# kkrt-labs/stwo-brainfuck

Hardware: AMD Instinct MI355X
Metric: trace cells committed+proved/sec (higher is better)
Workload: dtype u32 (M31 / QM31 modular arithmetic)

## Files before the change

stwo-brainfuck_amd/csrc/api.hip:

```cpp
#include "../../include/bfhip.h"
#include "ctx.h"
#include <cstdlib>
#include "host/circle.h"
#include "host/quotients.h"
#include "host/hash.h"
#include <cstdio>
#include <vector>
#include <algorithm>
#include <chrono>

using namespace bf;

static thread_local std::string g_err;
void bfhip_set_error(const std::string& s) { g_err = s; }

#define API_TRY try {
#define API_CTX(ctx) try { if (!(ctx)) throw HipError("null context"); (ctx)->c.bind();
#define API_CATCH } catch (const std::exception& e) { g_err = e.what(); return -1; } catch (...) { g_err = "unknown error"; return -1; }

namespace bf {

void Ctx::ensure_aux() { for (auto& a : aux) if (!a) BF_HIP(hipStreamCreateWithFlags(&a, hipStreamNonBlocking)); }
void Ctx::ensure_side() { if (!stream2) BF_HIP(hipStreamCreateWithFlags(&stream2, hipStreamNonBlocking)); }

// ... 817 lines not shown
        total = q_add(total, claimed[k]);
        reports[k] = check_report_init();
    }
    CheckLaunch launches[N_COMPONENTS];
    const CheckLaunch* d_launches = nullptr;
    CheckReportDev* d_reports = nullptr;
    {
        StageBatch sb(c);
        d_reports = c.stage(reports, N_COMPONENTS);
        for (int k = 0; k < N_COMPONENTS; k++) launches[k] = check_launch_of(k, log_sizes[k], rows[k], inter[k], el, claimed[k], d_reports + k);
        d_launches = c.stage(launches, N_COMPONENTS);
        sb.end();
    }
    {
        ProfScope ps(c.stream, "k_check_cells", 0);
        for (int k = 0; k < N_COMPONENTS; k++) check_constraints_launch(c.stream, k, d_launches + k, log_sizes[k]);
    }
    BF_HIP(hipGetLastError());
    c.read_back(reports, d_reports, sizeof reports);
    int32_t n_bad = 0;
    for (int k = 0; k < N_COMPONENTS; k++) { check_report_fill(out[k], reports[k], k, log_sizes[k], claimed[k]); n_bad += reports[k].n_bad_cells != 0; }
    logup_total_h[0] = total.a.a; logup_total_h[1] = total.a.b; logup_total_h[2] = total.b.a; logup_total_h[3] = total.b.b;
    if (n_bad_components) *n_bad_components = n_bad;
    return 0;
    API_CATCH
}
int32_t bfhip_accumulate_quotients(bfhip_ctx* ctx, uint32_t log_size, const uint32_t* const* cols_h, const uint32_t* col_shifts_h, uint32_t n_cols,
                                   const uint32_t* n_samples_h, const uint32_t* sample_points_h, const uint32_t* sample_values_h,
                                   const uint32_t random_coeff_h[4], uint32_t* const out_d[4]) {
    API_CTX(ctx)
    Ctx& c = ctx->c;
    if (log_size < 3 || log_size > c.tw_root_log + 1) throw HipError("accumulate_quotients: log_size outside the twiddle tree");
    std::vector<ColDesc> descs(n_cols);
    std::vector<std::vector<ColumnSample>> samples(n_cols);
    size_t si = 0;
    for (u32 k = 0; k < n_cols; k++) {
        descs[k] = ColDesc{cols_h[k], col_shifts_h ? col_shifts_h[k] : 0u, 0};
        if (descs[k].shift == 1) throw HipError("accumulate_quotients: column shift must be 0 or >= 2");
        for (u32 s = 0; s < n_samples_h[k]; s++, si++) {
            const uint32_t* p = sample_points_h + 8 * si;
            samples[k].push_back({PtQ{q_from_h(p), q_from_h(p + 4)}, q_from_h(sample_values_h + 4 * si)});
        }
    }
    std::vector<QuotientBatch> batches; std::vector<QuotientEntry> entries;
    build_quotient_batches(samples, q_from_h(random_coeff_h), batches, entries);
    quotient_entries_finish(batches.data(), batches.size(), entries.data(), descs.data());
    c.stage_checkpoint();
    QuotientArgs a{};
    a.batches = batches.empty() ? nullptr : c.stage(batches.data(), batches.size());
    a.entries = entries.empty() ? nullptr : c.stage(entries.data(), entries.size());
    a.n_batches = (u32)batches.size(); a.log = log_size; a.tw = c.d_tw; a.tw_total = 1u << c.tw_root_log;
    for (int w = 0; w < 4; w++) a.out[w] = out_d[w];
    const u32 blocks = quotient_groups_layout(&a, 1);
    accumulate_quotients(c.stream, c.stage(&a, 1), 1, blocks);
    BF_HIP(hipGetLastError());
    return 0;
    API_CATCH
}

}

#ifdef BFHIP_TEST_HOOKS
__global__ void __launch_bounds__(256) k_test_field_op(u32 op, const u32* __restrict__ a, const u32* __restrict__ b, u32* __restrict__ out, u32 n) {
    const u32 i = blockIdx.x * blockDim.x + threadIdx.x;
    if (i >= n) return;
    const u32 a0 = a[4 * i], a1 = a[4 * i + 1], a2 = a[4 * i + 2], a3 = a[4 * i + 3];
    const u32 b0 = b[4 * i], b1 = b[4 * i + 1], b2 = b[4 * i + 2], b3 = b[4 * i + 3];
    const u64 a64 = ((u64)a1 << 32) | a0;
    const Q31 x = q_make(a0, a1, a2, a3), y = q_make(b0, b1, b2, b3);
    Q31 r = q_zero();
    switch (op) {
        case 0: r.a.a = m_add(a0, b0); break;
        case 1: r.a.a = m_sub(a0, b0); break;
        case 2: r.a.a = m_mul(a0, b0); break;
        case 3: r.a.a = m_mul_pre2(a0, 2u * b0); break;
        case 4: r.a.a = m_mul_pow2(a0, b0 % 31u); break;
        case 5: r.a.a = m_inv(a0); break;
        case 6: r.a.a = m_red4(a64); break;
        case 7: r.a.a = m_canon(a64); break;
        case 8: r = q_mul(x, y); break;
        case 9: r = q_mul_const(x, q_const(y)); break;
        default: r = q_inv(x); break;
    }
    out[4 * i] = r.a.a; out[4 * i + 1] = r.a.b; out[4 * i + 2] = r.b.a; out[4 * i + 3] = r.b.b;
}
extern "C" int32_t bfhip_test_field_op(bfhip_ctx* ctx, uint32_t op, const uint32_t* a_d, const uint32_t* b_d, uint32_t* out_d, size_t n) {
    API_CTX(ctx)
    if (op > 10) throw HipError("bfhip_test_field_op: unknown op");
    if (!a_d || !b_d || !out_d) throw HipError("null argument");
    if (n == 0 || n > (size_t(1) << 28)) throw HipError("bfhip_test_field_op: n out of range");
    hipLaunchKernelGGL(k_test_field_op, dim3((u32)((n + 255) / 256)), dim3(256), 0, ctx->c.stream, op, a_d, b_d, out_d, (u32)n);
    BF_HIP(hipGetLastError());
    return 0;
    API_CATCH
}
extern "C" int32_t bfhip_test_constraint_group_rows(int32_t component, uint32_t log_size, uint32_t main_shift) {
    if (component < 0 || component >= N_COMPONENTS) { g_err = "unknown component"; return -1; }
    ConstraintLaunch L{};
    for (u32 j = 0; j < n_main_cols(component); j++) L.trace[j].shift = main_shift;
    for (u32 j = 0; j + 4 < 4 * n_logup_cols(component); j++) L.inter[j].shift = main_shift;
    L.log_size = log_size;
    return (int32_t)constraint_group_rows(L, component);
}
#endif
```

stwo-brainfuck_amd/csrc/kernels.h:

```cpp
#pragma once
#include <hip/hip_runtime.h>
#include "m31.h"
#include "air.h"
#include <string>
#include <vector>

struct bfhip_trace;

namespace bf {

struct ColDesc { const u32* ptr; u32 shift; u32 pad_; };

int prof_mode(hipStream_t s);
void prof_enable(hipStream_t s, int mode);
void prof_run_begin(hipStream_t s, const char* name);
void prof_run_end(hipStream_t s);
void prof_begin(hipStream_t s, const char* name, double bytes, double units, double aux = 0.0);
void prof_end(hipStream_t s);
void prof_reset(hipStream_t s);
std::string prof_report_json(const hipStream_t* streams, int n);
void prof_forget(hipStream_t s);
struct ProfScope {
    hipStream_t s; bool on;
    ProfScope(hipStream_t s_, const char* name, double bytes, double units = 0.0, bool dominant = false, double aux = 0.0) : s(s_) {
// ... 80 lines not shown
    const u32* src[4]; const u32* quot[4]; u32* dst[4]; uint4* tree[18];
    const u32* alpha8; const u32* itw; u32 tw_total, log, rfc, pad_;
    u32* counter; u32* chan; u32* alpha_out; u32* root_out;
};
void fri_layer(hipStream_t stream, const FriLayerArgs& a);
void grind_span(hipStream_t stream, const u32* d_digest, u64 base, u32 span, u32 pow_bits, unsigned long long* d_best, u32 mix_u64_conv);
void clock_probe_launch(hipStream_t stream, uint4* d_stamps, u32* d_sink, u32 blocks, u32 iters);
void clock_sampler_launch(hipStream_t stream, uint4* d_out, const u32* d_stop_alias, unsigned long long max_ticks);
void fill_mix(hipStream_t stream, u32* p, size_t n);
void channel_mix_root_draw(hipStream_t stream, u32* d_chan, const u32* d_root, u32* d_alpha8, u32* d_root_copy);

void merkle_layer_poseidon(hipStream_t stream, void* out, const void* prev, const ColDesc* d_cols, u32 ncols, u32 log, u32 out_shift = 0, u32 prev_shift = 0,
                           u32 first = 0, u32 count = 0);
void hades_once(hipStream_t stream, const u32* d_in24, u32* d_out24);

struct ConstraintLaunch {
    const u32* is_first; ColDesc trace[13]; ColDesc inter[12]; u32* acc[4]; Q31 coeff[12]; Lookups el; Q31 total_sum; u32 denom_inv[2]; u32 log_size;
    u32 overwrite;
    u32 row0, n_rows;
    const u32* inter_prev[4];
};
void eval_constraints(hipStream_t stream, int comp, const ConstraintLaunch* d_args, u32 log_size, u32 n_rows = 0, u32 group_rows = 0);
u32 constraint_group_rows(const ConstraintLaunch& L, int comp);
struct ConstraintClass { u32 n_comps, block0, group_rows, pad_; u32 comp[13]; u32 pad2_[3]; };
struct ConstraintBatch { u32 n_classes, total_blocks, pad_[2]; ConstraintClass cls[13]; };
void constraint_batch_init(ConstraintBatch& b, const ConstraintLaunch* launches, u32 n);
void eval_constraints_batch(hipStream_t stream, const ConstraintBatch* d_batch, const ConstraintBatch& h_batch, const ConstraintLaunch* d_args);
struct LogupLaunch {
    const u32* cols[13];
    u32* out_rep[8];
    u32* out_last[4];
    void* vrow; void* wloc; void* totals; void* claimed;
    Lookups el; u32 log_rows; int comp;
};
struct LogupItem { const u32* cols[13]; u32* out_rep[8]; u32* out_last[4]; uint4* vrow; uint4* wloc; uint4* totals; uint4* claimed; u32 log_rows; int comp; u32 nb; u32 pad_; };
struct LogupBatch { Lookups el; u32 n; u32 rows_blk0[14], scan_blk0[14], last_blk0[14]; u32 pad_; LogupItem item[13]; };
void logup_batch_init(LogupBatch& b, const Lookups& el, const LogupLaunch* L, u32 n);
void logup_batch_run(hipStream_t stream, const LogupBatch* d_batch, const LogupBatch& h_batch);
void broadcast16(hipStream_t stream, const u32* d_rows, u32* d_out, u32 n_cells);

struct CheckReportDev { u64 n_bad_cells, first_bad_cell; u64 bad_per_constraint[16]; u32 first_bad_constraint; u32 first_bad_value[4]; u32 pad_[3]; };
struct CheckLaunch { ColDesc trace[13]; ColDesc inter[12]; Lookups el; Q31 total_sum; u32 log_size; u32 pad_; CheckReportDev* report; };
void check_constraints_launch(hipStream_t stream, int comp, const CheckLaunch* d_args, u32 log_size);

void trace_columns(const bfhip_trace* t, const u32* cols[N_COMPONENTS][13], u32 log_sizes[N_COMPONENTS]);

struct EvalJob { const u32* coeffs; u32 log_n; u32 point; u32 factor_shift; u32 partial_off; u32 out_idx; u32 pad_; };
void eval_at_points(hipStream_t stream, const EvalJob* d_jobs, u32 n_jobs, u32 total_partials, const void* d_factors, void* d_partials, void* d_out);
struct QuotientBatch { C31 prx, pry, pix, piy; Q31 a_sum, b_sum, batch_coeff; u32 n_cols; C31 kden; u32 n_full; };
struct QuotientEntry { Q31 c; const u32* ptr; u32 shift; u32 col; };
void quotient_entries_finish(QuotientBatch* batches, size_t n_batches, QuotientEntry* entries, const ColDesc* cols);
struct QuotientArgs { const QuotientBatch* batches; const QuotientEntry* entries; u32 n_batches; u32 log; const u32* tw; u32 tw_total; u32* out[4]; u32 row0, n_rows; u32 block0, pad_; };
u32 quotient_groups_layout(QuotientArgs* h_groups, u32 n_groups);
void accumulate_quotients(hipStream_t stream, const QuotientArgs* d_groups, u32 n_groups, u32 total_blocks);
void fold_circle_into_line(hipStream_t stream, u32* const dst[4], const u32* const src[4], const u32* d_alpha8, const u32* itw, u32 tw_root_log, u32 log, bool fresh = false,
                           u32 first = 0, u32 count = 0);
void fold_line(hipStream_t stream, u32* const dst[4], const u32* const src[4], const u32* d_alpha8, const u32* itw, u32 tw_root_log, u32 log, u32 first = 0, u32 count = 0);
void fold_line_circle(hipStream_t stream, u32* const dst[4], const u32* const src[4], const u32* const quot[4], const u32* d_alpha8, const u32* itw, u32 tw_root_log, u32 log,
                      u32 first = 0, u32 count = 0);
void prev_row_copy(hipStream_t stream, u32* dst, const u32* src, u32 log_size);
struct GatherReq { const u32* base; u64 index; u32 out_off; u32 n_words; };
void gather_u32(hipStream_t stream, const GatherReq* d_req, u32 n, u32* d_out);
void accumulate(hipStream_t stream, u32* dst, const u32* src, u32 n);
struct AccumulateSizes { u32* dst[4]; const u32* src[12][4]; u32 log[12]; u32 n; };
void accumulate_sizes(hipStream_t stream, const AccumulateSizes& a);
void batch_inverse_m31(hipStream_t stream, const u32* src, u32* dst, u32 n);
void batch_inverse_qm31(hipStream_t stream, const u32* const src[4], u32* const dst[4], u32 n);
void bit_reverse(hipStream_t stream, const u32* src, u32* dst, u32 log);
void one_hot(hipStream_t stream, u32* dst, u32 n);

}
```

stwo-brainfuck_amd/csrc/m31.h:

```cpp
#pragma once
#include <cstdint>
#include <cstddef>

#if defined(__HIPCC__)
#include <hip/hip_runtime.h>
#define BF_HD __host__ __device__ __forceinline__
#else
#define BF_HD inline
#endif

namespace bf {

using u8 = uint8_t;
using u32 = uint32_t;
using u64 = uint64_t;

constexpr u32 P31 = 0x7fffffffu;

struct Conventions {
    u32 merkle_node_hash = 0;
    u32 mix_u64 = 0;
    u32 logup_mask_order = 0;
    u32 merkle_channel = 0;
};
// ... 16 lines not shown
BF_HD u32 m_mul_pre2(u32 a, u32 w2) {
    u64 p = (u64)a * w2;
    u32 s = (u32)(p >> 32) + ((u32)p >> 1); u32 t = s - P31; return t < s ? t : s;
}
BF_HD u32 m_mul_pow2(u32 a, u32 k) { return ((a << k) & P31) | (a >> (31u - k)); }
BF_HD u32 m_sqr(u32 a) { return m_mul(a, a); }
BF_HD u32 m_inv_pow2(u32 n) { return 1u << ((31u - n % 31u) % 31u); }
BF_HD u32 m_pow(u32 b, u32 e) { u32 r = 1; while (e) { if (e & 1) r = m_mul(r, b); b = m_mul(b, b); e >>= 1; } return r; }
BF_HD u32 m_sqn(u32 x, int n) { for (int i = 0; i < n; i++) x = m_sqr(x); return x; }
BF_HD u32 m_inv(u32 x) {
    u32 t0 = m_mul(m_sqn(x, 2), x);
    u32 t1 = m_mul(m_sqr(t0), t0);
    u32 t2 = m_mul(m_sqn(t1, 3), t0);
    u32 t3 = m_mul(m_sqr(t2), t0);
    u32 t4 = m_mul(m_sqn(t3, 8), t3);
    u32 t5 = m_mul(m_sqn(t4, 8), t3);
    return m_mul(m_sqn(t5, 7), t2);
}

struct C31 { u32 a, b; };
BF_HD C31 c_add(C31 x, C31 y) { return {m_add(x.a, y.a), m_add(x.b, y.b)}; }
BF_HD C31 c_sub(C31 x, C31 y) { return {m_sub(x.a, y.a), m_sub(x.b, y.b)}; }
BF_HD C31 c_neg(C31 x) { return {m_neg(x.a), m_neg(x.b)}; }
BF_HD C31 c_mul(C31 x, C31 y) { return {m_sub(m_mul(x.a, y.a), m_mul(x.b, y.b)), m_add(m_mul(x.a, y.b), m_mul(x.b, y.a))}; }
BF_HD C31 c_mulm(C31 x, u32 y) { return {m_mul(x.a, y), m_mul(x.b, y)}; }
BF_HD C31 c_mulR(C31 x) { return {m_sub(m_add(x.a, x.a), x.b), m_add(x.a, m_add(x.b, x.b))}; }
BF_HD C31 c_inv(C31 x) { u32 n = m_inv(m_add(m_sqr(x.a), m_sqr(x.b))); return {m_mul(x.a, n), m_neg(m_mul(x.b, n))}; }

struct Q31 { C31 a, b; };
BF_HD Q31 q_make(u32 a0, u32 a1, u32 a2, u32 a3) { return {{a0, a1}, {a2, a3}}; }
BF_HD Q31 q_zero() { return {{0, 0}, {0, 0}}; }
BF_HD Q31 q_one() { return {{1, 0}, {0, 0}}; }
BF_HD Q31 q_from_m(u32 x) { return {{x, 0}, {0, 0}}; }
BF_HD Q31 q_add(Q31 x, Q31 y) { return {c_add(x.a, y.a), c_add(x.b, y.b)}; }
BF_HD Q31 q_sub(Q31 x, Q31 y) { return {c_sub(x.a, y.a), c_sub(x.b, y.b)}; }
BF_HD Q31 q_neg(Q31 x) { return {c_neg(x.a), c_neg(x.b)}; }
BF_HD Q31 q_mul(Q31 x, Q31 y) { return {c_add(c_mul(x.a, y.a), c_mulR(c_mul(x.b, y.b))), c_add(c_mul(x.a, y.b), c_mul(x.b, y.a))}; }
BF_HD Q31 q_mulm(Q31 x, u32 y) { return {c_mulm(x.a, y), c_mulm(x.b, y)}; }
struct QConst { u32 c0, c1, c2, c3, e0, e1, nc1, nc3, ne1; };
BF_HD QConst q_const(Q31 y) {
    const C31 e = c_mulR(y.b);
    return {y.a.a, y.a.b, y.b.a, y.b.b, e.a, e.b, P31 - y.a.b, P31 - y.b.b, P31 - e.b};
}
BF_HD u32 m_red4(u64 x) {
    const u64 t = ((x >> 32) << 1) + (u32)x;
    const u32 s = ((u32)t & P31) + (u32)(t >> 31); const u32 d = s - P31; return d < s ? d : s;
}
BF_HD Q31 q_mul_const(Q31 x, const QConst& k) {
    const u64 a0 = x.a.a, a1 = x.a.b, b0 = x.b.a, b1 = x.b.b;
    return q_make(m_red4(a0 * k.c0 + a1 * k.nc1 + b0 * k.e0 + b1 * k.ne1), m_red4(a0 * k.c1 + a1 * k.c0 + b0 * k.e1 + b1 * k.e0),
                  m_red4(a0 * k.c2 + a1 * k.nc3 + b0 * k.c0 + b1 * k.nc1), m_red4(a0 * k.c3 + a1 * k.c2 + b0 * k.c1 + b1 * k.c0));
}
BF_HD Q31 q_mulc(Q31 x, C31 y) { return {c_mul(x.a, y), c_mul(x.b, y)}; }
BF_HD Q31 q_addm(Q31 x, u32 y) { x.a.a = m_add(x.a.a, y); return x; }
BF_HD Q31 q_subm(Q31 x, u32 y) { x.a.a = m_sub(x.a.a, y); return x; }
BF_HD Q31 q_conj(Q31 x) { return {x.a, c_neg(x.b)}; }
BF_HD Q31 q_inv(Q31 x) { C31 d = c_inv(c_sub(c_mul(x.a, x.a), c_mulR(c_mul(x.b, x.b)))); return {c_mul(x.a, d), c_neg(c_mul(x.b, d))}; }
BF_HD bool q_eq(Q31 x, Q31 y) { return x.a.a == y.a.a && x.a.b == y.a.b && x.b.a == y.b.a && x.b.b == y.b.b; }
BF_HD bool q_is_zero(Q31 x) { return (x.a.a | x.a.b | x.b.a | x.b.b) == 0; }
BF_HD Q31 q_pow(Q31 b, u64 e) { Q31 r = q_one(); while (e) { if (e & 1) r = q_mul(r, b); b = q_mul(b, b); e >>= 1; } return r; }

BF_HD u32 bit_rev(u32 i, u32 log) {
#if defined(__HIP_DEVICE_COMPILE__)
    return log ? (__brev(i) >> (32 - log)) : 0;
#else
    u32 r = 0; for (u32 k = 0; k < log; k++) r |= ((i >> k) & 1u) << (log - 1 - k); return r;
#endif
}

}
```

stwo-brainfuck_amd/csrc/prover.hip:

```cpp
#include <atomic>
#include "../../include/bfhip.h"
#include "ctx.h"
#include "host/circle.h"
#include "host/quotients.h"
#include "host/proof.h"
#include "host/verifier.h"
#include <map>
#include <set>
#include <chrono>
#include <algorithm>
#include <cstdio>
#include <functional>
#include <mutex>

namespace bf {

void build_tables_device(Ctx& c, const std::vector<u32> trace7_soa[7], u32 n, const std::vector<u32>& code, const std::function<u32*(size_t)>& alloc,
                         std::vector<std::vector<u32*>>& cols_out, u32 log_sizes_out[13]);

static constexpr u32 OWNER_ALL = 0xFFFFFFFFu;

struct DCol {
    u32* ptr = nullptr; u32 log_size = 0; u32 shift = 0;
    u32 lc = 0;
// ... 1236 lines not shown
                g.descs.push_back(flat[k].col.desc());
                ColSamples cs{};
                for (size_t s = 0; s < pts.size(); s++) { cs.point[cs.n] = pts[s]; cs.value[cs.n] = q_zero(); cs.n++; }
                g.cols.push_back(cs); g.src.push_back({flat[k].tree, flat[k].idx});
            }
            groups.push_back(std::move(g));
            i = j;
        }
        return groups;
    }
    static void quotient_constants(QuotientGroup& g, const std::vector<PtQ>& points, const StarkProof* pf, Q31 random_coeff,
                                   std::vector<QuotientBatch>& batches, std::vector<QuotientEntry>& entries) {
        if (pf)
            for (size_t k = 0; k < g.cols.size(); k++)
                for (u32 s = 0; s < g.cols[k].n; s++) g.cols[k].value[s] = pf->sampled_values[g.src[k].first][g.src[k].second][s];
        batches.clear(); entries.clear();
        build_quotient_batches_indexed(g.cols.data(), g.cols.size(), points, random_coeff, batches, entries);
        quotient_entries_finish(batches.data(), batches.size(), entries.data(), g.descs.data());
    }
    QuotientRun compute_quotients(const std::vector<DTree>& trees, const std::vector<std::vector<std::vector<u32>>>& mask, const std::vector<PtQ>& points,
                                  const StarkProof* pf, Q31 random_coeff, std::vector<LevelWait>* q_waits, Mailbox* mb0 = nullptr, Mailbox* mb1 = nullptr) {
        QuotientRun qr;
        qr.groups = quotient_groups(trees, mask);
        mark("quotient columns sorted");
        const bool pipelined = (c.overlap & 2u) && q_waits && !sharded() && c.conv.merkle_channel == 0;
        const bool early_first = !pipelined && !sharded();
        std::vector<QuotientArgs> launches;
        std::vector<QuotientBatch> batches; std::vector<QuotientEntry> entries;
        auto stage_group = [&](QuotientGroup& g, Mailbox* m) {
            quotient_constants(g, points, pf, random_coeff, batches, entries);
            const bool sl = slice_log(g.log);
            DSecure q; q.log_size = g.log; q.lc = sl ? lc() : 0;
            for (int w = 0; w < 4; w++) q.c[w] = sl ? alloc_slice(g.log) : c.alloc_u32(size_t(1) << g.log);
            QuotientArgs a{};
            if (sl) { a.row0 = (u32)slice_first(g.log); a.n_rows = (u32)slice_cells(g.log); }
            a.batches = batches.empty() ? nullptr : c.stage(batches.data(), batches.size());
            a.entries = entries.empty() ? nullptr : c.stage(entries.data(), entries.size());
            if (m) { g.n_batches = batches.size(); g.n_entries = entries.size(); g.h_batches = a.batches ? m->host(a.batches) : nullptr; g.h_entries = a.entries ? m->host(a.entries) : nullptr; }
            a.n_batches = (u32)batches.size(); a.log = g.log; a.tw = c.d_tw; a.tw_total = 1u << c.tw_root_log;
            for (int w = 0; w < 4; w++) a.out[w] = q.c[w];
            launches.push_back(a);
            qr.out.push_back(q);
        };
        c.stage_checkpoint();
        size_t launched = 0;
        if (early_first && !qr.groups.empty()) {
            u32 nblocks = 0; const QuotientArgs* d_first = nullptr;
            stage_blocks(mb0, [&] {
                stage_group(qr.groups[0], mb0);
                nblocks = quotient_groups_layout(&launches[0], 1);
                d_first = c.stage(&launches[0], 1);
            });
            if (mb0) BF_HIP(hipEventRecord(c.ev[4], c.stream));
            accumulate_quotients(c.stream, d_first, 1, nblocks);
            mark("largest quotient group launched");
            launched = 1;
        }
        if (launched < qr.groups.size()) {
            std::vector<std::pair<u32, u32>> ranges;
            std::vector<u32> blocks;
            const QuotientArgs* d_groups = nullptr;
            stage_blocks(mb1, [&] {
                for (size_t g = launched; g < qr.groups.size(); g++) stage_group(qr.groups[g], mb1);
                u32 g = (u32)launched;
                if (pipelined) while (g < launches.size() && launches[g].log >= 19) { ranges.push_back({g, 1u}); g++; }
                if (g < launches.size()) ranges.push_back({g, (u32)launches.size() - g});
                for (auto& r : ranges) blocks.push_back(quotient_groups_layout(launches.data() + r.first, r.second));
                d_groups = c.stage(launches.data(), launches.size());
            });
            for (size_t k = 0; k < ranges.size(); k++) {
                accumulate_quotients(c.stream, d_groups + ranges[k].first, ranges[k].second, blocks[k]);
                if (pipelined) { hipEvent_t e = c.next_event(); BF_HIP(hipEventRecord(e, c.stream)); q_waits->push_back({(int)launches[ranges[k].first].log, e}); }
            }
        }
        BF_HIP(hipGetLastError());
        return qr;
    }
    void quotients_fill(QuotientRun& qr, const std::vector<PtQ>& points, const StarkProof& pf, Q31 random_coeff, Mailbox* mb0, Mailbox* mb1) {
        std::vector<QuotientBatch> batches; std::vector<QuotientEntry> entries;
        for (size_t gi = 0; gi < qr.groups.size(); gi++) {
            QuotientGroup& g = qr.groups[gi];
            quotient_constants(g, points, &pf, random_coeff, batches, entries);
            if (batches.size() != g.n_batches || entries.size() != g.n_entries) throw HipError("quotients: the batch structure changed between enqueue and fill");
            if (g.n_batches) memcpy(g.h_batches, batches.data(), batches.size() * sizeof(QuotientBatch));
            if (g.n_entries) memcpy(g.h_entries, entries.data(), entries.size() * sizeof(QuotientEntry));
            if (gi == 0) mb0->post();
        }
        mb1->post();
    }

    static std::vector<size_t> fold_queries(const std::vector<size_t>& q, u32 n) {
        std::vector<size_t> o;
        for (size_t x : q) { size_t y = x >> n; if (o.empty() || o.back() != y) o.push_back(y); }
        return o;
    }
    static void positions_and_witness(const std::vector<size_t>& queries, std::vector<size_t>& positions, std::vector<size_t>& witness_pos) {
        size_t i = 0;
        while (i < queries.size()) {
            size_t j = i;
            while (j < queries.size() && (queries[j] >> 1) == (queries[i] >> 1)) j++;
            size_t start = (queries[i] >> 1) << 1, qi = i;
            for (size_t pos = start; pos < start + 2; pos++) {
                positions.push_back(pos);
                if (qi < j && queries[qi] == pos) { qi++; continue; }
                witness_pos.push_back(pos);
            }
            i = j;
        }
    }
    Finisher gather_secure_deferred(Gather& g, const DSecure& s, const std::vector<size_t>& pos, std::vector<Q31>* out) {
        size_t first = g.n_words;
        for (size_t p : pos) for (int w = 0; w < 4; w++) g.add(s.c[w], p, s.mine(p, c.shard.rank));
        size_t n = pos.size();
        return [first, n, out](const std::vector<u32>& d) { for (size_t k = 0; k < n; k++) out->push_back(q_make(d[first + 4 * k], d[first + 4 * k + 1], d[first + 4 * k + 2], d[first + 4 * k + 3])); };
    }
    std::vector<Q31> gather_secure(const DSecure& s, const std::vector<size_t>& pos) {
        Gather g;
        for (size_t p : pos) for (int w = 0; w < 4; w++) g.add(s.c[w], p, s.mine(p, c.shard.rank));
        auto d = g.run(c);
        std::vector<Q31> out;
        for (size_t k = 0; k < pos.size(); k++) out.push_back(q_make(d[4 * k], d[4 * k + 1], d[4 * k + 2], d[4 * k + 3]));
        return out;
    }
    static std::vector<DCol> secure_cols(const DSecure& s) {
// ... 512 lines not shown
```

stwo-brainfuck_amd/csrc/quotient.hip:

```cpp
#include <algorithm>
#include "kernels.h"
#include <stdexcept>

namespace bf {

__device__ __forceinline__ Q31 ld_q(const uint4* p, size_t i) { uint4 v = p[i]; return q_make(v.x, v.y, v.z, v.w); }
__device__ __forceinline__ uint4 pk_q(Q31 q) { return make_uint4(q.a.a, q.a.b, q.b.a, q.b.b); }

static constexpr u32 EAP_CHUNK_LOG = 12;

__global__ void __launch_bounds__(256) k_eval_at_point_stage1(const EvalJob* __restrict__ jobs, u32 n_jobs, const uint4* __restrict__ factors, uint4* __restrict__ partials) {
    u32 lo_j = 0, hi_j = n_jobs;
    while (hi_j - lo_j > 1) { u32 mid = (lo_j + hi_j) >> 1; if (jobs[mid].partial_off <= blockIdx.x) lo_j = mid; else hi_j = mid; }
    const EvalJob job = jobs[lo_j];
    const u32 n = 1u << job.log_n;
    const u32 chunk = blockIdx.x - job.partial_off;
    __shared__ uint4 s_w[16];
    __shared__ uint4 s_p[256];
    const uint4* F = factors + (size_t)job.point * 32 + job.factor_shift;
    const u32 t = threadIdx.x;
    if (t < 16) {
        Q31 w = q_one();
        for (u32 b = 0; b < 4; b++) if ((t >> b) & 1) w = q_mul(w, ld_q(F, b));
        s_w[t] = pk_q(w);
    }
    __syncthreads();
    const u32 base = (chunk << EAP_CHUNK_LOG) + t * 16;
    Q31 acc = q_zero();
    if (base < n) {
        if (n >= 16) {
            const uint4* src = reinterpret_cast<const uint4*>(job.coeffs + base);
            u64 a64[4] = {0, 0, 0, 0};
#pragma unroll
            for (u32 v4 = 0; v4 < 4; v4++) {
                const uint4 c = src[v4];
                const u32 cv[4] = {c.x, c.y, c.z, c.w};
#pragma unroll
                for (u32 j = 0; j < 4; j++) {
                    const u32 idx = v4 * 4 + j;
                    if (idx % 4 == 0 && idx) { a64[0] = m_fold(a64[0]); a64[1] = m_fold(a64[1]); a64[2] = m_fold(a64[2]); a64[3] = m_fold(a64[3]); }
                    const Q31 w = ld_q(s_w, idx);
                    a64[0] += (u64)w.a.a * cv[j]; a64[1] += (u64)w.a.b * cv[j]; a64[2] += (u64)w.b.a * cv[j]; a64[3] += (u64)w.b.b * cv[j];
                }
            }
            acc = q_make(m_red4(a64[0]), m_red4(a64[1]), m_red4(a64[2]), m_red4(a64[3]));
        } else {
            for (u32 k = 0; k < n; k++) acc = q_add(acc, q_mulm(ld_q(s_w, k), job.coeffs[k]));
        }
    }
    s_p[t] = pk_q(acc);
    __syncthreads();
    for (u32 b = 0; b < 8; b++) {
        u32 half = 128u >> b;
// ... 9 lines not shown
    }
    if (t == 0) partials[(size_t)job.partial_off + chunk] = s_p[0];
}

__global__ void __launch_bounds__(256) k_eval_at_point_stage2(const EvalJob* __restrict__ jobs, const uint4* __restrict__ factors, const uint4* __restrict__ partials, uint4* __restrict__ out) {
    const EvalJob job = jobs[blockIdx.x];
    const u32 nchunks = job.log_n > EAP_CHUNK_LOG ? 1u << (job.log_n - EAP_CHUNK_LOG) : 1u;
    const uint4* F = factors + (size_t)job.point * 32 + job.factor_shift;
    const uint4* p = partials + job.partial_off;
    __shared__ uint4 s[256];
    const u32 t = threadIdx.x;
    u32 lanes = nchunks < 256 ? nchunks : 256;
    u32 per_log = 0; while ((lanes << per_log) < nchunks) per_log++;
    Q31 acc = q_zero();
    if (t < lanes) {
        u32 per = 1u << per_log;
        for (u32 k = 0; k < per; k++) {
            Q31 w = q_one();
            for (u32 b = 0; b < per_log; b++) if ((k >> b) & 1) w = q_mul(w, ld_q(F, EAP_CHUNK_LOG + b));
            acc = q_add(acc, q_mul(ld_q(p, ((size_t)t << per_log) + k), w));
        }
    }
    s[t] = pk_q(acc);
    __syncthreads();
    u32 lanes_log = 0; while ((1u << lanes_log) < lanes) lanes_log++;
    for (u32 b = 0; b < lanes_log; b++) {
        u32 half = lanes >> (b + 1);
        Q31 r; bool act = t < half;
        if (act) r = q_add(ld_q(s, 2 * t), q_mul_const(ld_q(s, 2 * t + 1), q_const(ld_q(F, EAP_CHUNK_LOG + per_log + b))));
        __syncthreads();
        if (act) s[t] = pk_q(r);
        __syncthreads();
    }
    if (t == 0) out[job.out_idx] = s[0];
}

void eval_at_points(hipStream_t stream, const EvalJob* d_jobs, u32 n_jobs, u32 total_partials, const void* d_factors, void* d_partials, void* d_out) {
    if (!n_jobs) return;
    hipLaunchKernelGGL(k_eval_at_point_stage1, dim3(total_partials), dim3(256), 0, stream, d_jobs, n_jobs, (const uint4*)d_factors, (uint4*)d_partials);
    hipLaunchKernelGGL(k_eval_at_point_stage2, dim3(n_jobs), dim3(256), 0, stream, d_jobs, (const uint4*)d_factors, (const uint4*)d_partials, (uint4*)d_out);
}

__device__ __forceinline__ void domain_point(const u32* __restrict__ tw, u32 tw_total, u32 log, u32 row, u32& x, u32& y) {
    const u32* t1 = tw + (tw_total - (1u << (log - 1)));
    u32 xv = t1[row >> 2];
    x = (row & 2) ? m_neg(xv) : xv;
    u32 h = row >> 1;
    u32 cx = t1[(h >> 2) * 2], cy = t1[(h >> 2) * 2 + 1];
    u32 sel = h & 3;
    u32 yv = sel == 0 ? cy : sel == 1 ? m_neg(cy) : sel == 2 ? m_neg(cx) : cx;
    y = (row & 1) ? m_neg(yv) : yv;
}

__global__ void __launch_bounds__(256) k_quotients(const QuotientArgs* __restrict__ groups, u32 n_groups) {
    u32 g = 0;
    while (g + 1 < n_groups && groups[g + 1].block0 <= blockIdx.x) g++;
    const QuotientArgs& a = groups[g];
    u32 row0 = ((blockIdx.x - a.block0) * blockDim.x + threadIdx.x) * 4;
    if (a.n_rows) { if (row0 >= a.n_rows) return; row0 += a.row0; }
    else if (row0 >= (1u << a.log)) return;
    u32 xv, yv;
    domain_point(a.tw, a.tw_total, a.log, row0, xv, yv);
    Q31 acc[4] = {q_zero(), q_zero(), q_zero(), q_zero()};
    u32 e = 0;
    for (u32 b = 0; b < a.n_batches; b++) {
        const QuotientBatch qb = ld_constant(a.batches + b);
        u64 n64[4][4], s64[4];
#pragma unroll
        for (int r = 0; r < 4; r++) { n64[r][0] = 0; n64[r][1] = 0; n64[r][2] = 0; n64[r][3] = 0; }
        s64[0] = 0; s64[1] = 0; s64[2] = 0; s64[3] = 0;
        const QuotientEntry* ent = a.entries + e;
        e += qb.n_cols;
        const u32 nf = qb.n_full, nr = qb.n_cols - qb.n_full;
        if (nf) {
            uint4 A[3], B[3];
            const u32 last = nf - 1;
            auto load3 = [&](uint4 (&buf)[3], u32 k) {
#pragma unroll
                for (u32 j = 0; j < 3; j++) buf[j] = ld16(as_global(ld_constant(&ent[min(k + j, last)].ptr)) + row0);
            };
            auto mac3 = [&](const uint4 (&buf)[3], u32 k) {
#pragma unroll
                for (int r = 0; r < 4; r++) { n64[r][0] = m_fold(n64[r][0]); n64[r][1] = m_fold(n64[r][1]); n64[r][2] = m_fold(n64[r][2]); n64[r][3] = m_fold(n64[r][3]); }
#pragma unroll
                for (u32 j = 0; j < 3; j++) {
                    if (k + j < nf) {
                        const Q31 cc = ld_constant(&ent[k + j].c);
                        const u32 vr[4] = {buf[j].x, buf[j].y, buf[j].z, buf[j].w};
#pragma unroll
                        for (int r = 0; r < 4; r++) { n64[r][0] += (u64)cc.a.a * vr[r]; n64[r][1] += (u64)cc.a.b * vr[r]; n64[r][2] += (u64)cc.b.a * vr[r]; n64[r][3] += (u64)cc.b.b * vr[r]; }
                    }
                }
            };
            load3(A, 0);
            for (u32 k = 0; k < nf; k += 6) {
                load3(B, k + 3);
                mac3(A, k);
                load3(A, k + 6);
                mac3(B, k + 3);
            }
        }
        if (nr) {
            const QuotientEntry* er = ent + nf;
            u32 A[3], B[3];
            const u32 last = nr - 1;
            auto load3 = [&](u32 (&buf)[3], u32 k) {
#pragma unroll
                for (u32 j = 0; j < 3; j++) { const u32 i = min(k + j, last); buf[j] = as_global(ld_constant(&er[i].ptr))[row0 >> ld_constant(&er[i].shift)]; }
            };
            auto mac3 = [&](const u32 (&buf)[3], u32 k) {
                s64[0] = m_fold(s64[0]); s64[1] = m_fold(s64[1]); s64[2] = m_fold(s64[2]); s64[3] = m_fold(s64[3]);
#pragma unroll
                for (u32 j = 0; j < 3; j++) {
                    if (k + j < nr) {
                        const Q31 cc = ld_constant(&er[k + j].c);
                        s64[0] += (u64)cc.a.a * buf[j]; s64[1] += (u64)cc.a.b * buf[j]; s64[2] += (u64)cc.b.a * buf[j]; s64[3] += (u64)cc.b.b * buf[j];
                    }
                }
            };
            load3(A, 0);
            for (u32 k = 0; k < nr; k += 6) {
                load3(B, k + 3);
                mac3(A, k);
                load3(A, k + 6);
                mac3(B, k + 3);
            }
        }
        const Q31 ay = q_mulm(qb.a_sum, yv);
        const Q31 line_p = q_add(qb.b_sum, ay), line_m = q_sub(qb.b_sum, ay);
        const C31 P = {m_mul(xv, qb.piy.a), m_mul(xv, qb.piy.b)}, Q = {m_mul(yv, qb.pix.a), m_mul(yv, qb.pix.b)};
        const C31 km = c_sub(qb.kden, P), kp = c_add(qb.kden, P);
        C31 den[4] = {c_add(km, Q), c_sub(km, Q), c_sub(kp, Q), c_add(kp, Q)};
        Q31 num[4]; u32 nrm[4];
#pragma unroll
        for (int r = 0; r < 4; r++) {
            num[r] = q_make(m_canon(m_fold(n64[r][0]) + m_fold(s64[0])), m_canon(m_fold(n64[r][1]) + m_fold(s64[1])),
                            m_canon(m_fold(n64[r][2]) + m_fold(s64[2])), m_canon(m_fold(n64[r][3]) + m_fold(s64[3])));
            num[r] = q_sub(num[r], (r == 0 || r == 3) ? line_p : line_m);
            nrm[r] = m_add(m_sqr(den[r].a), m_sqr(den[r].b));
        }
        u32 p01 = m_mul(nrm[0], nrm[1]), p012 = m_mul(p01, nrm[2]), inv_all = m_inv(m_mul(p012, nrm[3]));
        u32 i3 = m_mul(inv_all, p012), t3 = m_mul(inv_all, nrm[3]);
        u32 i2 = m_mul(t3, p01), t2 = m_mul(t3, nrm[2]);
        u32 i1 = m_mul(t2, nrm[0]), i0 = m_mul(t2, nrm[1]);
        u32 ninv[4] = {i0, i1, i2, i3};
#pragma unroll
        for (int r = 0; r < 4; r++) {
            C31 dinv = {m_mul(den[r].a, ninv[r]), m_neg(m_mul(den[r].b, ninv[r]))};
            Q31 term = q_mulc(num[r], dinv);
            acc[r] = b ? q_add(acc[r], term) : term;
        }
    }
    *reinterpret_cast<uint4*>(a.out[0] + row0) = make_uint4(acc[0].a.a, acc[1].a.a, acc[2].a.a, acc[3].a.a);
    *reinterpret_cast<uint4*>(a.out[1] + row0) = make_uint4(acc[0].a.b, acc[1].a.b, acc[2].a.b, acc[3].a.b);
    *reinterpret_cast<uint4*>(a.out[2] + row0) = make_uint4(acc[0].b.a, acc[1].b.a, acc[2].b.a, acc[3].b.a);
    *reinterpret_cast<uint4*>(a.out[3] + row0) = make_uint4(acc[0].b.b, acc[1].b.b, acc[2].b.b, acc[3].b.b);
}
void quotient_entries_finish(QuotientBatch* batches, size_t n_batches, QuotientEntry* entries, const ColDesc* cols) {
    for (size_t b = 0; b < n_batches; b++) {
        QuotientEntry* first = entries; QuotientEntry* last = entries + batches[b].n_cols;
        for (QuotientEntry* q = first; q != last; q++) { q->ptr = cols[q->col].ptr; q->shift = cols[q->col].shift; }
        batches[b].n_full = (u32)(std::stable_partition(first, last, [](const QuotientEntry& q) { return q.shift == 0; }) - first);
        entries = last;
    }
}
u32 quotient_groups_layout(QuotientArgs* h_groups, u32 n_groups) {
    u32 blocks = 0;
    for (u32 g = 0; g < n_groups; g++) {
        const u32 lanes = (h_groups[g].n_rows ? h_groups[g].n_rows : (1u << h_groups[g].log)) / 4;
        h_groups[g].block0 = blocks;
        blocks += (lanes + 255) / 256;
    }
    return blocks;
}
void accumulate_quotients(hipStream_t stream, const QuotientArgs* d_groups, u32 n_groups, u32 total_blocks) {
    if (!n_groups || !total_blocks) return;
    ProfScope ps(stream, "k_quotients", 0);
    hipLaunchKernelGGL(k_quotients, dim3(total_blocks), dim3(256), 0, stream, d_groups, n_groups);
}

__global__ void __launch_bounds__(256) k_fold_circle_into_line(u32* const d0, u32* const d1, u32* const d2, u32* const d3,
                                                               const u32* __restrict__ s0, const u32* __restrict__ s1, const u32* __restrict__ s2, const u32* __restrict__ s3,
                                                               const u32* __restrict__ alpha8, const u32* __restrict__ itw, u32 tw_total, u32 log, u32 fresh, u32 first, u32 count) {
    u32 i = blockIdx.x * blockDim.x + threadIdx.x;
    if (i >= count) return;
    i += first;
    const QConst alpha = q_const(q_make(alpha8[0], alpha8[1], alpha8[2], alpha8[3])), alpha_sq = q_const(q_make(alpha8[4], alpha8[5], alpha8[6], alpha8[7]));
    const u32* t1 = itw + (tw_total - (1u << (log - 1)));
    u32 cx = t1[(i >> 2) * 2], cy = t1[(i >> 2) * 2 + 1], sel = i & 3;
    u32 yinv = sel == 0 ? cy : sel == 1 ? m_neg(cy) : sel == 2 ? m_neg(cx) : cx;
    uint2 a0 = reinterpret_cast<const uint2*>(s0)[i], a1 = reinterpret_cast<const uint2*>(s1)[i], a2 = reinterpret_cast<const uint2*>(s2)[i], a3 = reinterpret_cast<const uint2*>(s3)[i];
    Q31 fp = q_make(a0.x, a1.x, a2.x, a3.x), fn = q_make(a0.y, a1.y, a2.y, a3.y);
    Q31 f0 = q_add(fp, fn), f1 = q_mulm(q_sub(fp, fn), yinv);
    Q31 fprime = q_add(q_mul_const(f1, alpha), f0);
    Q31 r = fprime;
    if (!fresh) { Q31 dst = q_make(d0[i], d1[i], d2[i], d3[i]); r = q_add(q_mul_const(dst, alpha_sq), fprime); }
    d0[i] = r.a.a; d1[i] = r.a.b; d2[i] = r.b.a; d3[i] = r.b.b;
}
__global__ void __launch_bounds__(256) k_fold_line(u32* __restrict__ d0, u32* __restrict__ d1, u32* __restrict__ d2, u32* __restrict__ d3,
                                                   const u32* __restrict__ s0, const u32* __restrict__ s1, const u32* __restrict__ s2, const u32* __restrict__ s3,
                                                   const u32* __restrict__ alpha8, const u32* __restrict__ itw, u32 tw_total, u32 log, u32 first, u32 count) {
    u32 i = blockIdx.x * blockDim.x + threadIdx.x;
    if (i >= count) return;
    i += first;
    const QConst alpha = q_const(q_make(alpha8[0], alpha8[1], alpha8[2], alpha8[3]));
    u32 xinv = itw[tw_total - (1u << log) + i];
    uint2 a0 = reinterpret_cast<const uint2*>(s0)[i], a1 = reinterpret_cast<const uint2*>(s1)[i], a2 = reinterpret_cast<const uint2*>(s2)[i], a3 = reinterpret_cast<const uint2*>(s3)[i];
    Q31 fx = q_make(a0.x, a1.x, a2.x, a3.x), fn = q_make(a0.y, a1.y, a2.y, a3.y);
    Q31 f0 = q_add(fx, fn), f1 = q_mulm(q_sub(fx, fn), xinv);
    Q31 r = q_add(f0, q_mul_const(f1, alpha));
    d0[i] = r.a.a; d1[i] = r.a.b; d2[i] = r.b.a; d3[i] = r.b.b;
}
__global__ void __launch_bounds__(256) k_fold_line_circle(u32* __restrict__ d0, u32* __restrict__ d1, u32* __restrict__ d2, u32* __restrict__ d3,
                                                          const u32* __restrict__ s0, const u32* __restrict__ s1, const u32* __restrict__ s2, const u32* __restrict__ s3,
                                                          const u32* __restrict__ q0, const u32* __restrict__ q1, const u32* __restrict__ q2, const u32* __restrict__ q3,
                                                          const u32* __restrict__ alpha8, const u32* __restrict__ itw, u32 tw_total, u32 log, u32 first, u32 count) {
    u32 i = blockIdx.x * blockDim.x + threadIdx.x;
    if (i >= count) return;
    i += first;
    const QConst alpha = q_const(q_make(alpha8[0], alpha8[1], alpha8[2], alpha8[3]));
    Q31 r;
    {
        const u32 xinv = itw[tw_total - (1u << log) + i];
        const uint2 a0 = reinterpret_cast<const uint2*>(s0)[i], a1 = reinterpret_cast<const uint2*>(s1)[i], a2 = reinterpret_cast<const uint2*>(s2)[i], a3 = reinterpret_cast<const uint2*>(s3)[i];
        const Q31 fx = q_make(a0.x, a1.x, a2.x, a3.x), fn = q_make(a0.y, a1.y, a2.y, a3.y);
        r = q_add(q_add(fx, fn), q_mul_const(q_mulm(q_sub(fx, fn), xinv), alpha));
    }
    if (q0) {
        const QConst alpha_sq = q_const(q_make(alpha8[4], alpha8[5], alpha8[6], alpha8[7]));
        const u32* t1 = itw + (tw_total - (1u << (log - 1)));
        const u32 cx = t1[(i >> 2) * 2], cy = t1[(i >> 2) * 2 + 1], sel = i & 3;
// ... 122 lines not shown
```

Measured before the change: 14.34 billion.

## Share one field inversion across multiple quotient batches per row

Adds a quotient kernel variant that runs Montgomery batch inversion over denominators from up to 4 sample batches, so each thread does one m_inv per chunk of batches instead of one per batch. It also adds lazy conjugate-multiply and norm helpers that skip intermediate reductions and negations. The cost is recomputing the denominators twice, more registers for the per-batch inverse arrays, and a new host-side max-batches parameter used to pick the template variant. The new path is on by default and can be turned off with an environment variable.

```diff
diff --git a/stwo-brainfuck_amd/csrc/api.hip b/stwo-brainfuck_amd/csrc/api.hip
--- a/stwo-brainfuck_amd/csrc/api.hip
+++ b/stwo-brainfuck_amd/csrc/api.hip
@@ -893,7 +893,7 @@
     a.n_batches = (u32)batches.size(); a.log = log_size; a.tw = c.d_tw; a.tw_total = 1u << c.tw_root_log;
     for (int w = 0; w < 4; w++) a.out[w] = out_d[w];
     const u32 blocks = quotient_groups_layout(&a, 1);
-    accumulate_quotients(c.stream, c.stage(&a, 1), 1, blocks);
+    accumulate_quotients(c.stream, c.stage(&a, 1), 1, blocks, a.n_batches);
     BF_HIP(hipGetLastError());
     return 0;
     API_CATCH
diff --git a/stwo-brainfuck_amd/csrc/kernels.h b/stwo-brainfuck_amd/csrc/kernels.h
--- a/stwo-brainfuck_amd/csrc/kernels.h
+++ b/stwo-brainfuck_amd/csrc/kernels.h
@@ -156,7 +156,8 @@
 void quotient_entries_finish(QuotientBatch* batches, size_t n_batches, QuotientEntry* entries, const ColDesc* cols);
 struct QuotientArgs { const QuotientBatch* batches; const QuotientEntry* entries; u32 n_batches; u32 log; const u32* tw; u32 tw_total; u32* out[4]; u32 row0, n_rows; u32 block0, pad_; };
 u32 quotient_groups_layout(QuotientArgs* h_groups, u32 n_groups);
-void accumulate_quotients(hipStream_t stream, const QuotientArgs* d_groups, u32 n_groups, u32 total_blocks);
+u32 quotient_max_batches(const QuotientArgs* h_groups, u32 n_groups);
+void accumulate_quotients(hipStream_t stream, const QuotientArgs* d_groups, u32 n_groups, u32 total_blocks, u32 max_batches = 0);
 void fold_circle_into_line(hipStream_t stream, u32* const dst[4], const u32* const src[4], const u32* d_alpha8, const u32* itw, u32 tw_root_log, u32 log, bool fresh = false,
                            u32 first = 0, u32 count = 0);
 void fold_line(hipStream_t stream, u32* const dst[4], const u32* const src[4], const u32* d_alpha8, const u32* itw, u32 tw_root_log, u32 log, u32 first = 0, u32 count = 0);
diff --git a/stwo-brainfuck_amd/csrc/m31.h b/stwo-brainfuck_amd/csrc/m31.h
--- a/stwo-brainfuck_amd/csrc/m31.h
+++ b/stwo-brainfuck_amd/csrc/m31.h
@@ -92,6 +92,12 @@
                   m_red4(a0 * k.c2 + a1 * k.nc3 + b0 * k.c0 + b1 * k.nc1), m_red4(a0 * k.c3 + a1 * k.c2 + b0 * k.c1 + b1 * k.c0));
 }
 BF_HD Q31 q_mulc(Q31 x, C31 y) { return {c_mul(x.a, y), c_mul(x.b, y)}; }
+BF_HD C31 c_mul_conj_lazy(C31 x, C31 y) {
+    const u64 nyb = P31 - y.b;
+    return {m_red4((u64)x.a * y.a + (u64)x.b * y.b), m_red4((u64)x.b * y.a + x.a * nyb)};
+}
+BF_HD Q31 q_mulc_conj_lazy(Q31 x, C31 y) { return {c_mul_conj_lazy(x.a, y), c_mul_conj_lazy(x.b, y)}; }
+BF_HD u32 c_norm_lazy(C31 x) { return m_red4((u64)x.a * x.a + (u64)x.b * x.b); }
 BF_HD Q31 q_addm(Q31 x, u32 y) { x.a.a = m_add(x.a.a, y); return x; }
 BF_HD Q31 q_subm(Q31 x, u32 y) { x.a.a = m_sub(x.a.a, y); return x; }
 BF_HD Q31 q_conj(Q31 x) { return {x.a, c_neg(x.b)}; }
diff --git a/stwo-brainfuck_amd/csrc/prover.hip b/stwo-brainfuck_amd/csrc/prover.hip
--- a/stwo-brainfuck_amd/csrc/prover.hip
+++ b/stwo-brainfuck_amd/csrc/prover.hip
@@ -1312,7 +1312,7 @@
                 d_first = c.stage(&launches[0], 1);
             });
             if (mb0) BF_HIP(hipEventRecord(c.ev[4], c.stream));
-            accumulate_quotients(c.stream, d_first, 1, nblocks);
+            accumulate_quotients(c.stream, d_first, 1, nblocks, launches[0].n_batches);
             mark("largest quotient group launched");
             launched = 1;
         }
@@ -1329,7 +1329,7 @@
                 d_groups = c.stage(launches.data(), launches.size());
             });
             for (size_t k = 0; k < ranges.size(); k++) {
-                accumulate_quotients(c.stream, d_groups + ranges[k].first, ranges[k].second, blocks[k]);
+                accumulate_quotients(c.stream, d_groups + ranges[k].first, ranges[k].second, blocks[k], quotient_max_batches(launches.data() + ranges[k].first, ranges[k].second));
                 if (pipelined) { hipEvent_t e = c.next_event(); BF_HIP(hipEventRecord(e, c.stream)); q_waits->push_back({(int)launches[ranges[k].first].log, e}); }
             }
         }
diff --git a/stwo-brainfuck_amd/csrc/quotient.hip b/stwo-brainfuck_amd/csrc/quotient.hip
--- a/stwo-brainfuck_amd/csrc/quotient.hip
+++ b/stwo-brainfuck_amd/csrc/quotient.hip
@@ -1,4 +1,5 @@
 #include <algorithm>
+#include <cstdlib>
 #include "kernels.h"
 #include <stdexcept>
 
@@ -114,7 +115,148 @@
     y = (row & 1) ? m_neg(yv) : yv;
 }
 
-__global__ void __launch_bounds__(256) k_quotients(const QuotientArgs* __restrict__ groups, u32 n_groups) {
+__device__ __forceinline__ void quotient_numerators(const QuotientEntry* ent, u32 nf, u32 nr, u32 row0, u64 (&n64)[4][4], u64 (&s64)[4]) {
+#pragma unroll
+    for (int r = 0; r < 4; r++) { n64[r][0] = 0; n64[r][1] = 0; n64[r][2] = 0; n64[r][3] = 0; }
+    s64[0] = 0; s64[1] = 0; s64[2] = 0; s64[3] = 0;
+    if (nf) {
+        uint4 A[3], B[3];
+        const u32 last = nf - 1;
+        auto load3 = [&](uint4 (&buf)[3], u32 k) {
+#pragma unroll
+            for (u32 j = 0; j < 3; j++) buf[j] = ld16(as_global(ld_constant(&ent[min(k + j, last)].ptr)) + row0);
+        };
+        auto mac3 = [&](const uint4 (&buf)[3], u32 k) {
+#pragma unroll
+            for (int r = 0; r < 4; r++) { n64[r][0] = m_fold(n64[r][0]); n64[r][1] = m_fold(n64[r][1]); n64[r][2] = m_fold(n64[r][2]); n64[r][3] = m_fold(n64[r][3]); }
+#pragma unroll
+            for (u32 j = 0; j < 3; j++) {
+                if (k + j < nf) {
+                    const Q31 cc = ld_constant(&ent[k + j].c);
+                    const u32 vr[4] = {buf[j].x, buf[j].y, buf[j].z, buf[j].w};
+#pragma unroll
+                    for (int r = 0; r < 4; r++) { n64[r][0] += (u64)cc.a.a * vr[r]; n64[r][1] += (u64)cc.a.b * vr[r]; n64[r][2] += (u64)cc.b.a * vr[r]; n64[r][3] += (u64)cc.b.b * vr[r]; }
+                }
+            }
+        };
+        load3(A, 0);
+        for (u32 k = 0; k < nf; k += 6) {
+            load3(B, k + 3);
+            mac3(A, k);
+            load3(A, k + 6);
+            mac3(B, k + 3);
+        }
+    }
+    if (nr) {
+        const QuotientEntry* er = ent + nf;
+        u32 A[3], B[3];
+        const u32 last = nr - 1;
+        auto load3 = [&](u32 (&buf)[3], u32 k) {
+#pragma unroll
+            for (u32 j = 0; j < 3; j++) { const u32 i = min(k + j, last); buf[j] = as_global(ld_constant(&er[i].ptr))[row0 >> ld_constant(&er[i].shift)]; }
+        };
+        auto mac3 = [&](const u32 (&buf)[3], u32 k) {
+            s64[0] = m_fold(s64[0]); s64[1] = m_fold(s64[1]); s64[2] = m_fold(s64[2]); s64[3] = m_fold(s64[3]);
+#pragma unroll
+            for (u32 j = 0; j < 3; j++) {
+                if (k + j < nr) {
+                    const Q31 cc = ld_constant(&er[k + j].c);
+                    s64[0] += (u64)cc.a.a * buf[j]; s64[1] += (u64)cc.a.b * buf[j]; s64[2] += (u64)cc.b.a * buf[j]; s64[3] += (u64)cc.b.b * buf[j];
+                }
+            }
+        };
+        load3(A, 0);
+        for (u32 k = 0; k < nr; k += 6) {
+            load3(B, k + 3);
+            mac3(A, k);
+            load3(A, k + 6);
+            mac3(B, k + 3);
+        }
+    }
+}
+__device__ __forceinline__ void quotient_dens(C31 kden, C31 pix, C31 piy, u32 xv, u32 yv, C31 (&den)[4]) {
+    const C31 P = {m_mul(xv, piy.a), m_mul(xv, piy.b)}, Q = {m_mul(yv, pix.a), m_mul(yv, pix.b)};
+    const C31 km = c_sub(kden, P), kp = c_add(kden, P);
+    den[0] = c_add(km, Q); den[1] = c_sub(km, Q); den[2] = c_sub(kp, Q); den[3] = c_add(kp, Q);
+}
+__device__ __forceinline__ void quotient_nums(const QuotientBatch& qb, u32 yv, const u64 (&n64)[4][4], const u64 (&s64)[4], Q31 (&num)[4]) {
+    const Q31 ay = q_mulm(qb.a_sum, yv);
+    const Q31 line_p = q_add(qb.b_sum, ay), line_m = q_sub(qb.b_sum, ay);
+#pragma unroll
+    for (int r = 0; r < 4; r++) {
+        num[r] = q_make(m_canon(m_fold(n64[r][0]) + m_fold(s64[0])), m_canon(m_fold(n64[r][1]) + m_fold(s64[1])),
+                        m_canon(m_fold(n64[r][2]) + m_fold(s64[2])), m_canon(m_fold(n64[r][3]) + m_fold(s64[3])));
+        num[r] = q_sub(num[r], (r == 0 || r == 3) ? line_p : line_m);
+    }
+}
+__device__ __forceinline__ void quotient_store(const QuotientArgs& a, u32 row0, const Q31 (&acc)[4]) {
+    *reinterpret_cast<uint4*>(a.out[0] + row0) = make_uint4(acc[0].a.a, acc[1].a.a, acc[2].a.a, acc[3].a.a);
+    *reinterpret_cast<uint4*>(a.out[1] + row0) = make_uint4(acc[0].a.b, acc[1].a.b, acc[2].a.b, acc[3].a.b);
+    *reinterpret_cast<uint4*>(a.out[2] + row0) = make_uint4(acc[0].b.a, acc[1].b.a, acc[2].b.a, acc[3].b.a);
+    *reinterpret_cast<uint4*>(a.out[3] + row0) = make_uint4(acc[0].b.b, acc[1].b.b, acc[2].b.b, acc[3].b.b);
+}
+
+template <int MAXU>
+__global__ void __launch_bounds__(256) k_quotients_shared(const QuotientArgs* __restrict__ groups, u32 n_groups) {
+    u32 g = 0;
+    while (g + 1 < n_groups && groups[g + 1].block0 <= blockIdx.x) g++;
+    const QuotientArgs& a = groups[g];
+    u32 row0 = ((blockIdx.x - a.block0) * blockDim.x + threadIdx.x) * 4;
+    if (a.n_rows) { if (row0 >= a.n_rows) return; row0 += a.row0; }
+    else if (row0 >= (1u << a.log)) return;
+    u32 xv, yv;
+    domain_point(a.tw, a.tw_total, a.log, row0, xv, yv);
+    Q31 acc[4] = {q_zero(), q_zero(), q_zero(), q_zero()};
+    u32 e = 0;
+    for (u32 b0 = 0; b0 < a.n_batches; b0 += MAXU) {
+        const u32 nu = min((u32)MAXU, a.n_batches - b0);
+        u32 nrm[MAXU][4], pre[MAXU][4], ninv[MAXU][4];
+        u32 run = 1;
+#pragma unroll
+        for (u32 u = 0; u < MAXU; u++) {
+            if (u < nu) {
+                const QuotientBatch* pb = a.batches + b0 + u;
+                C31 den[4];
+                quotient_dens(ld_constant(&pb->kden), ld_constant(&pb->pix), ld_constant(&pb->piy), xv, yv, den);
+#pragma unroll
+                for (int r = 0; r < 4; r++) { nrm[u][r] = c_norm_lazy(den[r]); pre[u][r] = run; run = (u | r) ? m_mul(run, nrm[u][r]) : nrm[u][r]; }
+            }
+        }
+        u32 inv = m_inv(run);
+#pragma unroll
+        for (int u = MAXU - 1; u >= 0; u--) {
+            if ((u32)u < nu) {
+#pragma unroll
+                for (int r = 3; r >= 0; r--) {
+                    if (u | r) { ninv[u][r] = m_mul(inv, pre[u][r]); inv = m_mul(inv, nrm[u][r]); }
+                    else ninv[u][r] = inv;
+                }
+            }
+        }
+        for (u32 u = 0; u < nu; u++) {
+            const QuotientBatch qb = ld_constant(a.batches + b0 + u);
+            u64 n64[4][4], s64[4];
+            quotient_numerators(a.entries + e, qb.n_full, qb.n_cols - qb.n_full, row0, n64, s64);
+            e += qb.n_cols;
+            C31 den[4]; Q31 num[4];
+            quotient_dens(qb.kden, qb.pix, qb.piy, xv, yv, den);
+            quotient_nums(qb, yv, n64, s64, num);
+#pragma unroll
+            for (int r = 0; r < 4; r++) {
+                const C31 dn = {m_mul(den[r].a, ninv[0][r]), m_mul(den[r].b, ninv[0][r])};
+                const Q31 term = q_mulc_conj_lazy(num[r], dn);
+                acc[r] = (b0 | u) ? q_add(acc[r], term) : term;
+            }
+#pragma unroll
+            for (u32 k = 0; k + 1 < MAXU; k++)
+#pragma unroll
+                for (int r = 0; r < 4; r++) ninv[k][r] = ninv[k + 1][r];
+        }
+    }
+    quotient_store(a, row0, acc);
+}
+template <bool LAZY>
+__global__ void __launch_bounds__(256) k_quotients_per_batch(const QuotientArgs* __restrict__ groups, u32 n_groups) {
     u32 g = 0;
     while (g + 1 < n_groups && groups[g + 1].block0 <= blockIdx.x) g++;
     const QuotientArgs& a = groups[g];
@@ -128,79 +270,13 @@
     for (u32 b = 0; b < a.n_batches; b++) {
         const QuotientBatch qb = ld_constant(a.batches + b);
         u64 n64[4][4], s64[4];
-#pragma unroll
-        for (int r = 0; r < 4; r++) { n64[r][0] = 0; n64[r][1] = 0; n64[r][2] = 0; n64[r][3] = 0; }
-        s64[0] = 0; s64[1] = 0; s64[2] = 0; s64[3] = 0;
-        const QuotientEntry* ent = a.entries + e;
+        quotient_numerators(a.entries + e, qb.n_full, qb.n_cols - qb.n_full, row0, n64, s64);
         e += qb.n_cols;
-        const u32 nf = qb.n_full, nr = qb.n_cols - qb.n_full;
-        if (nf) {
-            uint4 A[3], B[3];
-            const u32 last = nf - 1;
-            auto load3 = [&](uint4 (&buf)[3], u32 k) {
-#pragma unroll
-                for (u32 j = 0; j < 3; j++) buf[j] = ld16(as_global(ld_constant(&ent[min(k + j, last)].ptr)) + row0);
-            };
-            auto mac3 = [&](const uint4 (&buf)[3], u32 k) {
-#pragma unroll
-                for (int r = 0; r < 4; r++) { n64[r][0] = m_fold(n64[r][0]); n64[r][1] = m_fold(n64[r][1]); n64[r][2] = m_fold(n64[r][2]); n64[r][3] = m_fold(n64[r][3]); }
-#pragma unroll
-                for (u32 j = 0; j < 3; j++) {
-                    if (k + j < nf) {
-                        const Q31 cc = ld_constant(&ent[k + j].c);
-                        const u32 vr[4] = {buf[j].x, buf[j].y, buf[j].z, buf[j].w};
-#pragma unroll
-                        for (int r = 0; r < 4; r++) { n64[r][0] += (u64)cc.a.a * vr[r]; n64[r][1] += (u64)cc.a.b * vr[r]; n64[r][2] += (u64)cc.b.a * vr[r]; n64[r][3] += (u64)cc.b.b * vr[r]; }
-                    }
-                }
-            };
-            load3(A, 0);
-            for (u32 k = 0; k < nf; k += 6) {
-                load3(B, k + 3);
-                mac3(A, k);
-                load3(A, k + 6);
-                mac3(B, k + 3);
-            }
-        }
-        if (nr) {
-            const QuotientEntry* er = ent + nf;
-            u32 A[3], B[3];
-            const u32 last = nr - 1;
-            auto load3 = [&](u32 (&buf)[3], u32 k) {
-#pragma unroll
-                for (u32 j = 0; j < 3; j++) { const u32 i = min(k + j, last); buf[j] = as_global(ld_constant(&er[i].ptr))[row0 >> ld_constant(&er[i].shift)]; }
-            };
-            auto mac3 = [&](const u32 (&buf)[3], u32 k) {
-                s64[0] = m_fold(s64[0]); s64[1] = m_fold(s64[1]); s64[2] = m_fold(s64[2]); s64[3] = m_fold(s64[3]);
-#pragma unroll
-                for (u32 j = 0; j < 3; j++) {
-                    if (k + j < nr) {
-                        const Q31 cc = ld_constant(&er[k + j].c);
-                        s64[0] += (u64)cc.a.a * buf[j]; s64[1] += (u64)cc.a.b * buf[j]; s64[2] += (u64)cc.b.a * buf[j]; s64[3] += (u64)cc.b.b * buf[j];
-                    }
-                }
-            };
-            load3(A, 0);
-            for (u32 k = 0; k < nr; k += 6) {
-                load3(B, k + 3);
-                mac3(A, k);
-                load3(A, k + 6);
-                mac3(B, k + 3);
-            }
-        }
-        const Q31 ay = q_mulm(qb.a_sum, yv);
-        const Q31 line_p = q_add(qb.b_sum, ay), line_m = q_sub(qb.b_sum, ay);
-        const C31 P = {m_mul(xv, qb.piy.a), m_mul(xv, qb.piy.b)}, Q = {m_mul(yv, qb.pix.a), m_mul(yv, qb.pix.b)};
-        const C31 km = c_sub(qb.kden, P), kp = c_add(qb.kden, P);
-        C31 den[4] = {c_add(km, Q), c_sub(km, Q), c_sub(kp, Q), c_add(kp, Q)};
-        Q31 num[4]; u32 nrm[4];
-#pragma unroll
-        for (int r = 0; r < 4; r++) {
-            num[r] = q_make(m_canon(m_fold(n64[r][0]) + m_fold(s64[0])), m_canon(m_fold(n64[r][1]) + m_fold(s64[1])),
-                            m_canon(m_fold(n64[r][2]) + m_fold(s64[2])), m_canon(m_fold(n64[r][3]) + m_fold(s64[3])));
-            num[r] = q_sub(num[r], (r == 0 || r == 3) ? line_p : line_m);
-            nrm[r] = m_add(m_sqr(den[r].a), m_sqr(den[r].b));
-        }
+        C31 den[4]; Q31 num[4]; u32 nrm[4];
+        quotient_dens(qb.kden, qb.pix, qb.piy, xv, yv, den);
+        quotient_nums(qb, yv, n64, s64, num);
+#pragma unroll
+        for (int r = 0; r < 4; r++) nrm[r] = LAZY ? c_norm_lazy(den[r]) : m_add(m_sqr(den[r].a), m_sqr(den[r].b));
         u32 p01 = m_mul(nrm[0], nrm[1]), p012 = m_mul(p01, nrm[2]), inv_all = m_inv(m_mul(p012, nrm[3]));
         u32 i3 = m_mul(inv_all, p012), t3 = m_mul(inv_all, nrm[3]);
         u32 i2 = m_mul(t3, p01), t2 = m_mul(t3, nrm[2]);
@@ -208,15 +284,13 @@
         u32 ninv[4] = {i0, i1, i2, i3};
 #pragma unroll
         for (int r = 0; r < 4; r++) {
-            C31 dinv = {m_mul(den[r].a, ninv[r]), m_neg(m_mul(den[r].b, ninv[r]))};
-            Q31 term = q_mulc(num[r], dinv);
+            Q31 term;
+            if (LAZY) term = q_mulc_conj_lazy(num[r], C31{m_mul(den[r].a, ninv[r]), m_mul(den[r].b, ninv[r])});
+            else term = q_mulc(num[r], C31{m_mul(den[r].a, ninv[r]), m_neg(m_mul(den[r].b, ninv[r]))});
             acc[r] = b ? q_add(acc[r], term) : term;
         }
     }
-    *reinterpret_cast<uint4*>(a.out[0] + row0) = make_uint4(acc[0].a.a, acc[1].a.a, acc[2].a.a, acc[3].a.a);
-    *reinterpret_cast<uint4*>(a.out[1] + row0) = make_uint4(acc[0].a.b, acc[1].a.b, acc[2].a.b, acc[3].a.b);
-    *reinterpret_cast<uint4*>(a.out[2] + row0) = make_uint4(acc[0].b.a, acc[1].b.a, acc[2].b.a, acc[3].b.a);
-    *reinterpret_cast<uint4*>(a.out[3] + row0) = make_uint4(acc[0].b.b, acc[1].b.b, acc[2].b.b, acc[3].b.b);
+    quotient_store(a, row0, acc);
 }
 void quotient_entries_finish(QuotientBatch* batches, size_t n_batches, QuotientEntry* entries, const ColDesc* cols) {
     for (size_t b = 0; b < n_batches; b++) {
@@ -235,10 +309,20 @@
     }
     return blocks;
 }
-void accumulate_quotients(hipStream_t stream, const QuotientArgs* d_groups, u32 n_groups, u32 total_blocks) {
+u32 quotient_max_batches(const QuotientArgs* h_groups, u32 n_groups) {
+    u32 m = 0;
+    for (u32 g = 0; g < n_groups; g++) m = std::max(m, h_groups[g].n_batches);
+    return m;
+}
+void accumulate_quotients(hipStream_t stream, const QuotientArgs* d_groups, u32 n_groups, u32 total_blocks, u32 max_batches) {
     if (!n_groups || !total_blocks) return;
+    static const bool shared = [] { const char* v = getenv("BFHIP_QUOTIENT_SHARED_INV"); return !v || v[0] != '0'; }();
     ProfScope ps(stream, "k_quotients", 0);
-    hipLaunchKernelGGL(k_quotients, dim3(total_blocks), dim3(256), 0, stream, d_groups, n_groups);
+    const dim3 grid(total_blocks), block(256);
+    if (!shared) hipLaunchKernelGGL(k_quotients_per_batch<false>, grid, block, 0, stream, d_groups, n_groups);
+    else if (max_batches == 1) hipLaunchKernelGGL(k_quotients_per_batch<true>, grid, block, 0, stream, d_groups, n_groups);
+    else if (max_batches == 2) hipLaunchKernelGGL(k_quotients_shared<2>, grid, block, 0, stream, d_groups, n_groups);
+    else hipLaunchKernelGGL(k_quotients_shared<4>, grid, block, 0, stream, d_groups, n_groups);
 }
 
 __global__ void __launch_bounds__(256) k_fold_circle_into_line(u32* const d0, u32* const d1, u32* const d2, u32* const d3,
```

New measurement: 14.41 billion (median of 6 runs). About the same (+0.5%).
